# OedonLestrange42/GNURadio-WiFI-ImageTransfer

Hardware: AMD Instinct MI355X
Metric: OFDM demod throughput (complex samples/s), 802.11a RX chain sync->LLR (higher is better)
Workload: dtype f32

## Files before the change

### gnuradio-wifi-imagetransfer_amd/csrc/wr_quad.h

```cpp
#pragma once
#include "wr_device.h"
#include "wr_kernels.h"
#include <type_traits>

namespace wr {

#define WR_QLDS_SCRATCH_EQ(EQ) ((EQ) == WIFIRX_EQ_COMB ? 768 : 1200)
#define WR_QLDS_H(S)       (S)
#define WR_QLDS_TW(S)      (WR_QLDS_H(S) + 512)
#define WR_QLDS_PREV(S)    (WR_QLDS_TW(S) + 192)
#define WR_QLDS_W(S)       (WR_QLDS_PREV(S) + 48)
#define WR_QLDS_PF(S)      (WR_QLDS_W(S))
#define WR_QLDS_STAT(S)    (WR_QLDS_PF(S) + 512)
#define WR_QLDS_FLOATS(S)  (WR_QLDS_STAT(S) + 16)
#define WR_QLDS_DH(S)      (WR_QLDS_FLOATS(S))
#define WR_QLDS_FLOATS_EQ(EQ) (WR_QLDS_FLOATS(WR_QLDS_SCRATCH_EQ(EQ)) + ((EQ) == WIFIRX_EQ_COMB ? 512 : 0))

typedef float wr_f2 __attribute__((ext_vector_type(2)));
__device__ __forceinline__ float2 load_global_f2(const float2* p)
{
#if defined(__HIP_DEVICE_COMPILE__)
    const wr_f2 v = __builtin_nontemporal_load(reinterpret_cast<const __attribute__((address_space(1))) wr_f2*>(reinterpret_cast<uintptr_t>(p)));
    return make_float2(v.x, v.y);
#else
// ... 631 lines not shown
__device__ __forceinline__ void store_piece(char* p, float4 v)
{
    __builtin_nontemporal_store(wr_f4v{ v.x, v.y, v.z, v.w }, reinterpret_cast<wr_f4v*>(p));
}
__device__ __forceinline__ void store_word(uint8_t* p, uint32_t v)
{
    *reinterpret_cast<uint32_t*>(p) = v;
}

template <int NB, bool OFF32 = false, bool BF = false>
__device__ __forceinline__ void store_bins_lines(const c32 (&Y)[4], const int (&carrier)[4], bool ok, int q,
                                                 uint8_t* __restrict__ idx, float* __restrict__ llr,
                                                 uint32_t row_o, uint32_t row_l, float* stage, int row, int r)
{
    static_assert(NB == 1 || NB == 2 || NB == 4 || NB == 6, "constellation");
    constexpr int VB = BF ? 2 : 4;
    constexpr int ROWB = 48 * VB * NB, IDX0 = NB <= 2 ? (BF ? 768 : 1536) : 4 * ROWB;
    char* srow = reinterpret_cast<char*>(stage) + row * ROWB;
    uint8_t* irow = reinterpret_cast<uint8_t*>(stage) + IDX0 + row * 48;
    __builtin_amdgcn_wave_barrier();
    if (NB <= 4) {
        constexpr int ESZ = VB * NB, DUMP_L = IDX0 + 192, DUMP_I = DUMP_L + 64 * ESZ;
        const int lane = 16 * row + r;
#pragma unroll
        for (int j = 0; j < 4; j++) {
            const bool data = carrier[j] >= 0;
            char* lw = data ? srow + ESZ * carrier[j] : reinterpret_cast<char*>(stage) + DUMP_L + ESZ * lane;
            uint8_t* iw = data ? irow + carrier[j] : reinterpret_cast<uint8_t*>(stage) + DUMP_I + lane;
            if constexpr (BF) {
                if (NB == 1)      *reinterpret_cast<uint16_t*>(lw) = bf16_of(Y[j].re);
                else if (NB == 2) *reinterpret_cast<uint32_t*>(lw) = bf16_pk(Y[j].re, Y[j].im);
                else              *reinterpret_cast<uint2*>(lw) = make_uint2(bf16_pk(Y[j].re, WR_T16_2 - __builtin_fabsf(Y[j].re)),
                                                                             bf16_pk(Y[j].im, WR_T16_2 - __builtin_fabsf(Y[j].im)));
            } else
            if (NB == 1)      *reinterpret_cast<float*>(lw) = Y[j].re;
            else if (NB == 2) *reinterpret_cast<float2*>(lw) = make_float2(Y[j].re, Y[j].im);
            else              *reinterpret_cast<float4*>(lw) = make_float4(Y[j].re, WR_T16_2 - __builtin_fabsf(Y[j].re), Y[j].im, WR_T16_2 - __builtin_fabsf(Y[j].im));
            *iw = decide(Y[j], NB);
        }
    } else
#pragma unroll
    for (int j = 0; j < 4; j++) {
        const uint64_t row_bits = j == 0 ? 0xF7C0ull : j == 1 ? 0xFDFFull : j == 2 ? 0xFF7Eull : 0x07DFull;
        if (!__builtin_amdgcn_inverse_ballot_w64(row_bits * 0x0001000100010001ull)) continue;
        const float are = __builtin_fabsf(Y[j].re), aim = __builtin_fabsf(Y[j].im);
        if constexpr (BF) {
            const uint32_t ci = (uint32_t)(carrier[j] + 48 * row);
            uint32_t l12;
            if (OFF32) asm volatile("v_mul_u32_u24 %0, 12, %1" : "=v"(l12) : "v"(ci));
            else       l12 = 12u * ci;
            uint32_t* l3 = reinterpret_cast<uint32_t*>(reinterpret_cast<char*>(stage) + l12);
            l3[0] = bf16_pk(Y[j].re, WR_T64_4 - are);
            l3[1] = bf16_pk(WR_T64_2 - __builtin_fabsf(are - WR_T64_4), Y[j].im);
            l3[2] = bf16_pk(WR_T64_4 - aim, WR_T64_2 - __builtin_fabsf(aim - WR_T64_4));
            reinterpret_cast<uint8_t*>(stage)[IDX0 + ci] = decide(Y[j], NB);
            continue;
        } else
        if (NB == 1)      *reinterpret_cast<float*>(srow + 4 * carrier[j]) = Y[j].re;
        else if (NB == 2) *reinterpret_cast<float2*>(srow + 8 * carrier[j]) = make_float2(Y[j].re, Y[j].im);
        else if (NB == 4) *reinterpret_cast<float4*>(srow + 16 * carrier[j]) = make_float4(Y[j].re, WR_T16_2 - are, Y[j].im, WR_T16_2 - aim);
        else if (OFF32) {
            const uint32_t ci = (uint32_t)(carrier[j] + 48 * row);
            uint32_t l24;
            asm volatile("v_mul_u32_u24 %0, 24, %1" : "=v"(l24) : "v"(ci));
            float2* l2 = reinterpret_cast<float2*>(reinterpret_cast<char*>(stage) + l24);
            l2[0] = make_float2(Y[j].re, WR_T64_4 - are);
            l2[1] = make_float2(WR_T64_2 - __builtin_fabsf(are - WR_T64_4), Y[j].im);
            l2[2] = make_float2(WR_T64_4 - aim, WR_T64_2 - __builtin_fabsf(aim - WR_T64_4));
            reinterpret_cast<uint8_t*>(stage)[IDX0 + ci] = decide(Y[j], NB);
            continue;
        } else {
            float2* l2 = reinterpret_cast<float2*>(srow + 24 * carrier[j]);
            l2[0] = make_float2(Y[j].re, WR_T64_4 - are);
            l2[1] = make_float2(WR_T64_2 - __builtin_fabsf(are - WR_T64_4), Y[j].im);
            l2[2] = make_float2(WR_T64_4 - aim, WR_T64_2 - __builtin_fabsf(aim - WR_T64_4));
        }
        irow[carrier[j]] = decide(Y[j], NB);
    }
    __builtin_amdgcn_wave_barrier();
    constexpr int PPR = 3 * VB * NB;
    constexpr int NK = (PPR + 15) / 16, TAIL = PPR - 16 * (NK - 1);
#define WR_PIECE(k) (*reinterpret_cast<const float4*>(srow + 256 * (k) + 16 * (((k) == NK - 1 && TAIL == 8) ? (r & 7) : r)))
    const float4 p0 = WR_PIECE(0);
    float4 p1 = p0, p2 = p0, p3 = p0, p4 = p0;
    if (NK > 1) p1 = WR_PIECE(1);
    if (NK > 2) p2 = WR_PIECE(2);
    if (NK > 3) p3 = WR_PIECE(3);
    if (NK > 4) p4 = WR_PIECE(4);
#undef WR_PIECE
    const uint32_t d = reinterpret_cast<const uint32_t*>(irow)[r < 12 ? r : 0];
    __builtin_amdgcn_wave_barrier();
    if (ok) {
        char* const lb = reinterpret_cast<char*>(llr);
        const uint32_t lo = (row_l + (uint32_t)(q * 48 * NB)) * (uint32_t)VB + 16u * r;
        char* const lp = reinterpret_cast<char*>(llr) + (uint32_t)((row_l + (uint32_t)(q * 48 * NB)) * (uint32_t)VB + 16u * r);
#define WR_PIECE_AT(K) (OFF32 ? lb + (uint32_t)(lo + 256u * (K)) : lp + 256 * (K))
        if (NK > 1 || r < TAIL)            store_piece(lp, p0);
        if (NK > 2 || (NK == 2 && r < TAIL)) store_piece(WR_PIECE_AT(1), p1);
        if (NK > 3 || (NK == 3 && r < TAIL)) store_piece(WR_PIECE_AT(2), p2);
        if (NK > 4 || (NK == 4 && r < TAIL)) store_piece(WR_PIECE_AT(3), p3);
        if (NK == 5 && r < TAIL)             store_piece(WR_PIECE_AT(4), p4);
#undef WR_PIECE_AT
        if (r < 12) store_word(idx + (row_o + (uint32_t)(q * 48) + 4u * r), d);
    }
}

template <int NB, bool OFF32 = false, bool BF = false>
__device__ __forceinline__ void store_rows_x(const c32 (&Y)[4], const int (&carrier)[4], bool ok, int q,
                                             uint8_t* __restrict__ idx, float* __restrict__ llr, float2* __restrict__ car,
                                             bool has_idx, bool has_llr, bool has_car, bool csi, const float* Wl,
                                             uint32_t row_o, uint32_t row_l, float* stage, int row, int r)
{
    static_assert(NB == 1 || NB == 2 || NB == 4 || NB == 6, "constellation");
    constexpr int VB = BF ? 2 : 4;
    constexpr int ROWB = 48 * VB * NB, IDX0 = NB <= 2 ? (BF ? 768 : 1536) : 4 * ROWB;
    constexpr int PPR = 3 * VB * NB;
    constexpr int NK = (PPR + 15) / 16, TAIL = PPR - 16 * (NK - 1);
    char* srow = reinterpret_cast<char*>(stage) + row * ROWB;
    uint8_t* irow = reinterpret_cast<uint8_t*>(stage) + IDX0 + row * 48;
    float4 p0 = make_float4(0.0f, 0.0f, 0.0f, 0.0f), p1 = p0;
    if (has_idx || has_llr) {
        float w[4] = { 1.0f, 1.0f, 1.0f, 1.0f };
        if (csi) {
#pragma unroll
            for (int j = 0; j < 4; j++) w[j] = Wl[64 * j];
        }
        __builtin_amdgcn_wave_barrier();
#pragma unroll
        for (int j = 0; j < 4; j++) {
            const uint64_t row_bits = j == 0 ? 0xF7C0ull : j == 1 ? 0xFDFFull : j == 2 ? 0xFF7Eull : 0x07DFull;
            if (!__builtin_amdgcn_inverse_ballot_w64(row_bits * 0x0001000100010001ull)) continue;
            const float are = __builtin_fabsf(Y[j].re), aim = __builtin_fabsf(Y[j].im);
#define WR_WT(v) (csi ? (v) * w[j] : (v))
            if constexpr (BF) {
                if (NB == 1)      *reinterpret_cast<uint16_t*>(srow + 2 * carrier[j]) = bf16_of(WR_WT(Y[j].re));
                else if (NB == 2) *reinterpret_cast<uint32_t*>(srow + 4 * carrier[j]) = bf16_pk(WR_WT(Y[j].re), WR_WT(Y[j].im));
                else if (NB == 4) *reinterpret_cast<uint2*>(srow + 8 * carrier[j]) = make_uint2(bf16_pk(WR_WT(Y[j].re), WR_WT(WR_T16_2 - are)),
                                                                                                 bf16_pk(WR_WT(Y[j].im), WR_WT(WR_T16_2 - aim)));
                else {
                    uint32_t* l3 = reinterpret_cast<uint32_t*>(srow + 12 * carrier[j]);
                    l3[0] = bf16_pk(WR_WT(Y[j].re), WR_WT(WR_T64_4 - are));
                    l3[1] = bf16_pk(WR_WT(WR_T64_2 - __builtin_fabsf(are - WR_T64_4)), WR_WT(Y[j].im));
                    l3[2] = bf16_pk(WR_WT(WR_T64_4 - aim), WR_WT(WR_T64_2 - __builtin_fabsf(aim - WR_T64_4)));
                }
            } else
            if (NB == 1)      *reinterpret_cast<float*>(srow + 4 * carrier[j]) = WR_WT(Y[j].re);
            else if (NB == 2) *reinterpret_cast<float2*>(srow + 8 * carrier[j]) = make_float2(WR_WT(Y[j].re), WR_WT(Y[j].im));
            else if (NB == 4) *reinterpret_cast<float4*>(srow + 16 * carrier[j]) = make_float4(WR_WT(Y[j].re), WR_WT(WR_T16_2 - are), WR_WT(Y[j].im), WR_WT(WR_T16_2 - aim));
            else {
                float2* l2 = reinterpret_cast<float2*>(srow + 24 * carrier[j]);
                l2[0] = make_float2(WR_WT(Y[j].re), WR_WT(WR_T64_4 - are));
                l2[1] = make_float2(WR_WT(WR_T64_2 - __builtin_fabsf(are - WR_T64_4)), WR_WT(Y[j].im));
                l2[2] = make_float2(WR_WT(WR_T64_4 - aim), WR_WT(WR_T64_2 - __builtin_fabsf(aim - WR_T64_4)));
            }
#undef WR_WT
            irow[carrier[j]] = decide(Y[j], NB);
        }
        __builtin_amdgcn_wave_barrier();
#define WR_PIECE(k) (*reinterpret_cast<const float4*>(srow + 256 * (k) + 16 * (((k) == NK - 1 && TAIL == 8) ? (r & 7) : r)))
        p0 = WR_PIECE(0);
        float4 p2 = p0, p3 = p0, p4 = p0;
        p1 = p0;
        if (NK > 1) p1 = WR_PIECE(1);
        if (NK > 2) p2 = WR_PIECE(2);
        if (NK > 3) p3 = WR_PIECE(3);
        if (NK > 4) p4 = WR_PIECE(4);
#undef WR_PIECE
        const uint32_t d = reinterpret_cast<const uint32_t*>(irow)[r < 12 ? r : 0];
        __builtin_amdgcn_wave_barrier();
        if (ok) {
            if (has_llr) {
                char* const lb = reinterpret_cast<char*>(llr);
                const uint32_t lo = (row_l + (uint32_t)(q * 48 * NB)) * (uint32_t)VB + 16u * r;
                char* const lp = reinterpret_cast<char*>(llr) + (uint32_t)((row_l + (uint32_t)(q * 48 * NB)) * (uint32_t)VB + 16u * r);
#define WR_PIECE_AT(K) (OFF32 ? lb + (uint32_t)(lo + 256u * (K)) : lp + 256 * (K))
                if (NK > 1 || r < TAIL)            store_piece(lp, p0);
                if (NK > 2 || (NK == 2 && r < TAIL)) store_piece(WR_PIECE_AT(1), p1);
                if (NK > 3 || (NK == 3 && r < TAIL)) store_piece(WR_PIECE_AT(2), p2);
                if (NK > 4 || (NK == 4 && r < TAIL)) store_piece(WR_PIECE_AT(3), p3);
                if (NK == 5 && r < TAIL)             store_piece(WR_PIECE_AT(4), p4);
#undef WR_PIECE_AT
            }
            if (has_idx && r < 12) store_word(idx + (row_o + (uint32_t)(q * 48) + 4u * r), d);
        }
    }
    if (has_car) {
        constexpr bool QPSK_F32 = NB == 2 && !BF;
        if (!(QPSK_F32 && has_llr && !csi)) {
            char* crow = reinterpret_cast<char*>(stage) + row * 384;
            __builtin_amdgcn_wave_barrier();
#pragma unroll
            for (int j = 0; j < 4; j++) {
                const uint64_t row_bits = j == 0 ? 0xF7C0ull : j == 1 ? 0xFDFFull : j == 2 ? 0xFF7Eull : 0x07DFull;
                if (!__builtin_amdgcn_inverse_ballot_w64(row_bits * 0x0001000100010001ull)) continue;
                *reinterpret_cast<float2*>(crow + 8 * carrier[j]) = make_float2(Y[j].re, Y[j].im);
            }
            __builtin_amdgcn_wave_barrier();
            p0 = *reinterpret_cast<const float4*>(crow + 16 * r);
            p1 = *reinterpret_cast<const float4*>(crow + 256 + 16 * (r & 7));
            __builtin_amdgcn_wave_barrier();
        }
        if (ok) {
            if (OFF32) {
                char* const cb = reinterpret_cast<char*>(car);
                const uint32_t co = (row_o + (uint32_t)(q * 48)) * 8u + 16u * r;
                store_piece(cb + co, p0);
                if (r < 8) store_piece(cb + (uint32_t)(co + 256u), p1);
            } else {
                char* cp = reinterpret_cast<char*>(car) + (uint32_t)((row_o + (uint32_t)(q * 48)) * 8u + 16u * r);
                store_piece(cp, p0);
                if (r < 8) store_piece(cp + 256, p1);
            }
        }
    }
}

#define WR_HB_DATA_LO 0xFDFFF7C0u
#define WR_HB_DATA_HI 0x07DFFF7Eu

template <int NB, int B>
__device__ __forceinline__ bool decide_bit(c32 y)
{
    const float are = __builtin_fabsf(y.re), aim = __builtin_fabsf(y.im);
    if (NB == 1) return y.re > 0.0f;
    if (NB == 2) return B == 0 ? y.re > 0.0f : y.im > 0.0f;
    if (NB == 4) return B == 0 ? y.re > 0.0f : B == 1 ? are < WR_T16_2 : B == 2 ? y.im > 0.0f : aim < WR_T16_2;
    return B == 0 ? y.re > 0.0f : B == 1 ? are < WR_T64_4 : B == 2 ? (are < WR_T64_6) && (are > WR_T64_2)
         : B == 3 ? y.im > 0.0f : B == 4 ? aim < WR_T64_4 : (aim < WR_T64_6) && (aim > WR_T64_2);
}

template <int NB, int B>
__device__ __forceinline__ void plane_words(const c32 (&Y)[4], uint32_t& w0, uint32_t& w1)
{
    const uint64_t m0 = __ballot(decide_bit<NB, B>(Y[0])), m1 = __ballot(decide_bit<NB, B>(Y[1]));
    const uint64_t m2 = __ballot(decide_bit<NB, B>(Y[2])), m3 = __ballot(decide_bit<NB, B>(Y[3]));
    const uint32_t a0 = (uint32_t)m0, a1 = (uint32_t)m1, a2 = (uint32_t)m2, a3 = (uint32_t)m3;
    const uint32_t b0 = (uint32_t)(m0 >> 32), b1 = (uint32_t)(m1 >> 32), b2 = (uint32_t)(m2 >> 32), b3 = (uint32_t)(m3 >> 32);
#pragma unroll
    for (int f = 0; f < 4; f++) {
        const uint32_t p0 = f < 2 ? a0 : b0, p1 = f < 2 ? a1 : b1, p2 = f < 2 ? a2 : b2, p3 = f < 2 ? a3 : b3;
        uint32_t lo, hi;
        if (f & 1) {
            asm("s_pack_hh_b32_b16 %0, %1, %2" : "=s"(lo) : "s"(p0), "s"(p1));
            asm("s_pack_hh_b32_b16 %0, %1, %2" : "=s"(hi) : "s"(p2), "s"(p3));
        } else {
            asm("s_pack_ll_b32_b16 %0, %1, %2" : "=s"(lo) : "s"(p0), "s"(p1));
            asm("s_pack_ll_b32_b16 %0, %1, %2" : "=s"(hi) : "s"(p2), "s"(p3));
        }
        asm("v_writelane_b32 %0, %1, %2" : "+v"(w0) : "s"(lo & WR_HB_DATA_LO), "n"(16 * f));
        asm("v_writelane_b32 %0, %1, %2" : "+v"(w1) : "s"(hi & WR_HB_DATA_HI), "n"(16 * f));
    }
}

template <int NB>
__device__ __forceinline__ void store_hbits(const c32 (&Y)[4], bool ok, int q, uint32_t* __restrict__ hb, int r)
{
    uint32_t* dst = hb + (unsigned)(q * 2 * NB);
    if (NB == 1) {
        uint32_t w0 = 0, w1 = 0;
        plane_words<1, 0>(Y, w0, w1);
        if (ok && r == 0) *reinterpret_cast<uint2*>(dst) = make_uint2(w0, w1);
    } else {
        uint4 w = make_uint4(0u, 0u, 0u, 0u);
        plane_words<NB, 0>(Y, w.x, w.y);
        plane_words<NB, 1>(Y, w.z, w.w);
        if (ok && r == 0) *reinterpret_cast<uint4*>(dst) = w;
        if (NB >= 4) {
            plane_words<NB, 2>(Y, w.x, w.y);
            plane_words<NB, (NB >= 4 ? 3 : 0)>(Y, w.z, w.w);
            if (ok && r == 0) *reinterpret_cast<uint4*>(dst + 4) = w;
        }
        if (NB == 6) {
            plane_words<NB, (NB == 6 ? 4 : 0)>(Y, w.x, w.y);
            plane_words<NB, (NB == 6 ? 5 : 0)>(Y, w.z, w.w);
            if (ok && r == 0) *reinterpret_cast<uint4*>(dst + 8) = w;
        }
    }
}

__device__ __forceinline__ c32 point_of(unsigned idx, int n_bpsc)
{
    c32 p;
    if (n_bpsc == 1) { p.re = (idx & 1) ? 1.0f : -1.0f; p.im = 0.0f; return p; }
    if (n_bpsc == 2) {
        p.re = (idx & 1) ? WR_LEVEL_QPSK : -WR_LEVEL_QPSK;
        p.im = (idx & 2) ? WR_LEVEL_QPSK : -WR_LEVEL_QPSK;
        return p;
    }
    if (n_bpsc == 4) {
        const float l = WR_T16_2 * 0.5f;
        float ar = (idx & 2) ? l : 3.0f * l, ai = (idx & 8) ? l : 3.0f * l;
        p.re = (idx & 1) ? ar : -ar;
        p.im = (idx & 4) ? ai : -ai;
        return p;
    }
    const float l = WR_T64_2 * 0.5f;
    unsigned r = (idx >> 1) & 3, q = (idx >> 4) & 3;
    unsigned kr = ((r & 1) << 1) | (r >> 1), kq = ((q & 1) << 1) | (q >> 1);
    float ar = (kr == 0 ? 7.0f : kr == 1 ? 5.0f : kr == 2 ? 1.0f : 3.0f) * l;
    float ai = (kq == 0 ? 7.0f : kq == 1 ? 5.0f : kq == 2 ? 1.0f : 3.0f) * l;
    p.re = (idx & 1) ? ar : -ar;
    p.im = (idx & 8) ? ai : -ai;
    return p;
}

template <int EQ, bool HB, bool XK, bool BF = false>
__device__ __forceinline__ void frames_quad(const QuadSeed& seed, const DemodParams& prm, float* qlds, int lane,
                                            const DemodOut& dout)
{
    wifirx_frame* __restrict__ frames = dout.frames;
    uint8_t* __restrict__ idx_all = dout.idx;
    float* __restrict__ llr_all = dout.llr;
    float2* __restrict__ car_all = dout.carrier;
    float2* __restrict__ csi_all = dout.csi;
    float4* __restrict__ stat_all = dout.sym_stats;
    uint32_t* __restrict__ hb_all = dout.hbits;
    constexpr bool LMS = EQ == WIFIRX_EQ_LMS, COMB = EQ == WIFIRX_EQ_COMB, STA = EQ == WIFIRX_EQ_STA;
    constexpr int QS = WR_QLDS_SCRATCH_EQ(EQ);
    constexpr bool DIV = EQ != WIFIRX_EQ_LS;
    const int row = lane >> 4, r = lane & 15;
    const bool  has = seed.out >= 0 && seed.x != nullptr && seed.t >= 0;
    const long  t16 = seed.t - 16;
    const uint64_t has_m = __ballot(has);
    const int has_l = has_m ? (int)__builtin_ctzll(has_m) : 0;
    const uint64_t xv = has ? reinterpret_cast<uint64_t>(seed.x + t16) : 0ull;
    const uint64_t xf = ((uint64_t)(uint32_t)__builtin_amdgcn_readlane((int)(xv >> 32), has_l) << 32) |
                        (uint32_t)__builtin_amdgcn_readlane((int)xv, has_l);
    const float2* xb = has ? seed.x + t16 : reinterpret_cast<const float2*>(xf);
    const int   m_lo = has ? (int)(t16 < 0 ? -t16 : 0) : 0;
    const long  m_hi_l = seed.n_samp - t16;
    const int   m_hi = has ? (int)(m_hi_l > 0x7fffff00l ? 0x7fffff00l : m_hi_l) : 0;
    const int   L = (int)seed.L;
    const bool  lo_zero = __all(m_lo == 0 && L <= m_hi && (!has || m_hi >= 64));
    const int   out = (int)seed.out;
    const int   trig = (int)seed.t;
    const float cfo_c = seed.cfo_c, cfo_f = seed.cfo_f;
    const int   fs = seed.fs;
    uint32_t flags = seed.flags;
    bool alive = (out >= 0) && (flags & WIFIRX_F_SYNC);
    const double bw = prm.bandwidth, fc = prm.frequency;
    const double two_pi = 2 * 3.14159265358979323846;
    const double tag = (double)cfo_c - (double)cfo_f;
    const float eps0 = (float)(tag * bw / (two_pi * fc));
    const float er_scale = (float)(bw / (two_pi * fc * 80));
    float d_er = 0.0f;
    const double theta_d = (double)cfo_f - (double)cfo_c;
    const unsigned long long Qp = (unsigned long long)(long long)__builtin_rint(theta_d * WR_TWO_OVER_PI_D * 4611686018427387904.0);
    constexpr bool QP_LDS = EQ != WIFIRX_EQ_LS;
    constexpr int PVS = QP_LDS ? 6 : 4;
    uint2* const qpl = reinterpret_cast<uint2*>(qlds + WR_QLDS_PREV(WR_QLDS_SCRATCH_EQ(EQ))) + PVS * (lane >> 4) + 4;
    if (QP_LDS && (lane & 15) == 0) *qpl = make_uint2((uint32_t)Qp, (uint32_t)(Qp >> 32));
    c32 u16;
    {
        const unsigned long long q16 = Qp * 16ull;
        sp_sincos_q((uint32_t)(q16 >> 32), (uint32_t)q16, u16.im, u16.re);
    }
    c32 u80;
    {
        const unsigned long long q80 = Qp * 80ull;
        sp_sincos_q((uint32_t)(q80 >> 32), (uint32_t)q80, u80.im, u80.re);
    }
    c32 wbase = { 1.0f, 0.0f };
    const float rp_bpsk = sp_recip(1.0f);
    const float rp_qpsk = sp_recip(fma_(WR_LEVEL_QPSK, WR_LEVEL_QPSK, WR_LEVEL_QPSK * WR_LEVEL_QPSK));
    int n_sym = 0, n_bpsc = 1, n_out = 0, enc = 0, psdu_len = 0;
    bool have_signal = false, want_llr = false;
    float snr = 0.0f;

    float2* twl = reinterpret_cast<float2*>(qlds + WR_QLDS_TW(QS));
    if (row == 0) {
#pragma unroll
        for (int j = 1; j < 4; j++) {
            int e1 = (j * r) & 63, e2 = (j * (r & 3) * 4) & 63;
            twl[(j - 1) * 16 + r] = make_float2(WR_TWIDDLE64[2 * e1], WR_TWIDDLE64[2 * e1 + 1]);
            twl[(j + 2) * 16 + r] = make_float2(WR_TWIDDLE64[2 * e2], WR_TWIDDLE64[2 * e2 + 1]);
        }
    }
    float* stl = qlds + WR_QLDS_STAT(QS) + 4 * row;
    if (stat_all != nullptr && r < 4) stl[r] = 0.0f;
    float2* Hl = reinterpret_cast<float2*>(qlds + WR_QLDS_H(QS)) + lane;
    float2* pvl = reinterpret_cast<float2*>(qlds + WR_QLDS_PREV(QS)) + PVS * row;
    float* Wl = qlds + WR_QLDS_W(QS) + lane;
    float2* DHl = reinterpret_cast<float2*>(qlds + (COMB ? WR_QLDS_DH(QS) : WR_QLDS_H(QS))) + lane;
    float cw[4] = { 0.0f, 0.0f, 0.0f, 0.0f }, cu[4] = { 0.0f, 0.0f, 0.0f, 0.0f };
    if (COMB) {
#pragma unroll
        for (int j = 0; j < 4; j++) { cw[j] = WR_COMB_W[r + 16 * j]; cu[j] = WR_COMB_U[r + 16 * j]; }
    }
    auto sta_inv_of = [&](int j) __attribute__((always_inline)) -> float {
        const uint64_t m3 = j == 0 ? 0x0040ull : j == 3 ? 0x0400ull : 0ull;
        const uint64_t m4 = j == 0 ? 0x0080ull : j == 1 ? 0xC000ull : j == 2 ? 0x0006ull : 0x0200ull;
        float v = 0x1.99999ap-3f;
        v = __builtin_amdgcn_inverse_ballot_w64(m4 * 0x0001000100010001ull) ? 0.25f : v;
        if (m3) v = __builtin_amdgcn_inverse_ballot_w64(m3 * 0x0001000100010001ull) ? 0x1.555556p-2f : v;
        return v;
    };
    int carrier0[4];
#pragma unroll
    for (int j = 0; j < 4; j++) {
        const int i = r + 16 * j;
        const bool data = (i >= 6 && i <= 58 && i != 11 && i != 25 && i != 32 && i != 39 && i != 53);
        carrier0[j] = data ? (i - 6 - (i > 11) - (i > 25) - (i > 32) - (i > 39) - (i > 53)) : -1;
    }
    __builtin_amdgcn_wave_barrier();
    constexpr bool TP_PAD = EQ != WIFIRX_EQ_COMB;
    float2* ql = reinterpret_cast<float2*>(qlds) + (TP_PAD ? 144 * row : 128 * (row >> 1) + 16 * (row & 1));
    const int m4 = 4 * (r & 3), c2 = r >> 2;
    const size_t per = (size_t)prm.max_sym * 48;
    const uint64_t have_out = __ballot(out >= 0);
    const int out_base = have_out ? __builtin_amdgcn_readlane(out, (int)__builtin_ctzll(have_out)) : 0;
    const uint32_t row_o = out >= 0 ? (uint32_t)(out - out_base) * (uint32_t)per : 0u;
    const uint32_t row_l = row_o * prm.llr_bits;
    uint8_t* idx = idx_all ? idx_all + (size_t)out_base * per : nullptr;
    float*   llr = llr_all ? llr_all + (size_t)out_base * per * prm.llr_bits : nullptr;
    if constexpr (BF)
        llr = llr_all ? reinterpret_cast<float*>(reinterpret_cast<uint16_t*>(llr_all) + (size_t)out_base * per * prm.llr_bits) : nullptr;
    float2*  car = car_all ? car_all + (size_t)out_base * per : nullptr;
    const bool lines_ok = (reinterpret_cast<uintptr_t>(idx) & 3) == 0 && (reinterpret_cast<uintptr_t>(llr) & 15) == 0 && ((per * prm.llr_bits) & 3) == 0;

    uint64_t polw = WR_POLARITY_NEG_LO;
    int poln = 64;
    int polhi = 0;
    float t4 = WR_T4_64F[0];
    const float* t4_next = WR_T4_64F + 1;
    int s_end = 0;
    int nbu_all = 0;
    bool plain_all = false;
    bool x_idx = false, x_llr = false, x_car = false, x_csi = false;
    uint32_t pf_voff0 = 0, pf_voff1 = 0;
    const float2* pf_next = nullptr;
    int pf_end = 0;
    bool pf_row = false;
    int pf_nst = 0;
    const uint32_t pf_m0 = (uint32_t)__builtin_amdgcn_readfirstlane((int)(uint32_t)reinterpret_cast<uintptr_t>(qlds + WR_QLDS_PF(QS)));
    const uint32_t pf_m1 = (uint32_t)__builtin_amdgcn_readfirstlane((int)(pf_m0 + 1024u));
    auto pf_issue = [&](float dep) __attribute__((always_inline)) {
        asm volatile("s_mov_b32 m0, %0\n\ts_nop 0\n\tglobal_load_lds_dwordx4 %2, %4\n\t"
                     "s_mov_b32 m0, %1\n\ts_nop 0\n\tglobal_load_lds_dwordx4 %3, %4"
                     :: "s"(pf_m0), "s"(pf_m1), "v"(pf_voff0), "v"(pf_voff1), "s"(pf_next), "v"(dep) : "memory", "m0");
        pf_next += 80;
    };
    auto pf_setup = [&](uint64_t has_data, int s0) __attribute__((always_inline)) -> bool {
        const int first = (int)__builtin_ctzll(has_data);
        const bool mine = s_end > 3;
        pf_end = __builtin_amdgcn_readlane(s_end, first);
        pf_row = mine;
        const uint64_t xbv = reinterpret_cast<uint64_t>(xb);
        const uint64_t xref = ((uint64_t)(uint32_t)__builtin_amdgcn_readlane((int)(xbv >> 32), first) << 32) |
                              (uint32_t)__builtin_amdgcn_readlane((int)xbv, first);
        const int64_t dist = (int64_t)(xbv - xref) / (int64_t)sizeof(float2);
        if (!__all(!mine || (s_end == pf_end && dist >= 0 && dist < (1 << 26)))) return false;
        const int c_own = (int)dist + fs;
        const int c_ref = __builtin_amdgcn_readlane(c_own, first);
        const int c = mine ? c_own : c_ref;
        const int c0 = __builtin_amdgcn_readlane(c, 0), c1 = __builtin_amdgcn_readlane(c, 16);
        const int c2 = __builtin_amdgcn_readlane(c, 32), c3 = __builtin_amdgcn_readlane(c, 48);
        pf_voff0 = (uint32_t)((lane < 32 ? c0 : c1) + 2 * (lane & 31)) * 8u;
        pf_voff1 = (uint32_t)((lane < 32 ? c2 : c3) + 2 * (lane & 31)) * 8u;
        pf_next = reinterpret_cast<const float2*>(xref) + (128 + 80 * (s0 - 2) + 16);
        __builtin_amdgcn_wave_barrier();
        pf_issue(0.0f);
        asm volatile("s_waitcnt vmcnt(0)" ::: "memory");
        return true;
    };
    auto symbol = [&](auto data_c, auto nb_c, auto x_c, auto p_c, const int s) __attribute__((always_inline)) -> bool {
        constexpr bool DATA = decltype(data_c)::value;
        constexpr int NBC = decltype(nb_c)::value;
        constexpr bool XC = decltype(x_c)::value;
        constexpr bool PC = decltype(p_c)::value;
        const int off0 = fs + ((!DATA && s < 2) ? 64 * s : 128 + 80 * (s - 2) + 16);
        bool act;
        if (DATA) {
            act = PC ? pf_row : s < s_end;
        } else {
            act = alive && (s <= n_sym + 2);
            if (act && (off0 + 64 > L || (s > 2 && (s - 3) >= (int)prm.max_sym))) {
                flags |= WIFIRX_F_TRUNCATED;
                alive = false;
                act = false;
            }
        }
        if (!(DATA && PC) && !__any(act)) return false;

        c32 v[4], cur[4];
        {
            if (PC) {
                constexpr int NST = ((BF ? 6 : 12) * (NBC ? NBC : 1) + 15) / 16 + 1 + (HB ? ((NBC ? NBC : 1) + 1) / 2 : 0);
                if (XC) {
                    switch (pf_nst) {
#define WR_W(N) case N: asm volatile("s_waitcnt vmcnt(" #N ")" ::: "memory"); break;
                    WR_W(1) WR_W(2) WR_W(3) WR_W(4) WR_W(5) WR_W(6) WR_W(7) WR_W(8) WR_W(9) WR_W(10) WR_W(11)
#undef WR_W
                    default: asm volatile("s_waitcnt vmcnt(0)" ::: "memory"); break;
                    }
                } else
                asm volatile("s_waitcnt vmcnt(%0)" :: "n"(NST) : "memory");
                const float2* pb = reinterpret_cast<const float2*>(qlds + WR_QLDS_PF(QS)) + 64 * row + r;
#pragma unroll
                for (int j = 0; j < 4; j++) { const float2 t = pb[16 * j]; cur[j] = { t.x, t.y }; }
            } else
            if (NBC != 0 || lo_zero) {
                const float2* p = xb + ((act ? off0 : 0) + r);
#pragma unroll
                for (int j = 0; j < 4; j++) { const float2 t = load_global_f2(p + 16 * j); cur[j] = { t.x, t.y }; }
            } else {
#pragma unroll
                for (int j = 0; j < 4; j++) cur[j] = load_y(xb, off0 + r + 16 * j, m_lo, act ? m_hi : 0);
            }
        }
        {
            if ((!DATA && s < 2) || ((s - 1) & 7) == 0) {
                unsigned long long qp = Qp;
                if (DATA && QP_LDS) { const uint2 q2 = *qpl; qp = ((unsigned long long)q2.y << 32) | q2.x; }
                const unsigned long long ph = qp * (unsigned long long)(unsigned)(off0 + r);
                sp_sincos_q((uint32_t)(ph >> 32), (uint32_t)ph, wbase.im, wbase.re);
            } else {
                wbase = sp_cmul(wbase, u80);
            }
            c32 w = wbase;
#pragma unroll
            for (int j = 0; j < 4; j++) {
                v[j] = sp_cmul(cur[j], w);
                w = sp_cmul(w, u16);
            }
            if (PC && s + 1 < pf_end) pf_issue(v[3].re);
        }
        bfly4_reg(v[0], v[1], v[2], v[3]);
#pragma unroll
        for (int j = 0; j < 4; j++) {
            c32 y = v[0];
            if (j) { float2 w = twl[(j - 1) * 16 + r]; y = sp_cmul(v[j], c32{ w.x, w.y }); }
            ql[TP_PAD ? 33 * j + m4 + c2 : 32 * j + m4 + (j ^ c2)] = make_float2(y.re, y.im);
        }
        __builtin_amdgcn_wave_barrier();
#pragma unroll
        for (int j = 0; j < 4; j++) {
            float2 t = ql[TP_PAD ? 33 * c2 + m4 + j : 32 * c2 + m4 + (c2 ^ j)];
            v[j] = { t.x, t.y };
        }
        __builtin_amdgcn_wave_barrier();
        bfly4_reg(v[0], v[1], v[2], v[3]);
#pragma unroll
        for (int j = 0; j < 4; j++) {
            c32 y = v[0];
            if (j) { float2 w = twl[(j + 2) * 16 + r]; y = sp_cmul(v[j], c32{ w.x, w.y }); }
            ql[TP_PAD ? 33 * j + 4 * c2 + (r & 3) : 32 * j + 4 * c2 + (j ^ (r & 3))] = make_float2(y.re, y.im);
        }
        __builtin_amdgcn_wave_barrier();
#pragma unroll
        for (int j = 0; j < 4; j++) {
            float2 t = ql[TP_PAD ? 33 * c2 + m4 + j : 32 * c2 + m4 + (c2 ^ j)];
            v[j] = { t.x, t.y };
        }
        __builtin_amdgcn_wave_barrier();
        bfly4_reg(v[0], v[1], v[2], v[3]);
        c32 X[4] = { v[2], v[3], v[0], v[1] };

        {
            const float kf = t4 * (eps0 + d_er);
            if (DATA) { t4 = PC ? load_const_f(t4_next) : *t4_next; t4_next++; }
            else { t4 = WR_T4_64F[s + 1]; t4_next = WR_T4_64F + (s + 2); }
            c32 b;
            sp_sincos_small(kf * (float)(r - 16), b.im, b.re);
            const c32 b0 = row_bcast<0>(b), step = { b0.re, -b0.im };
            const c32 q0 = sp_cmul(b, b0), q2 = sp_cmul(b, step), q3 = sp_cmul(q2, step);
            X[0] = sp_cmul(X[0], q0);
            X[1] = sp_cmul(X[1], b);
            X[2] = sp_cmul(X[2], q2);
            X[3] = sp_cmul(X[3], q3);
        }
        c32 X11 = row_bcast<11>(X[0]), X25 = row_bcast<9>(X[1]), X39 = row_bcast<7>(X[2]), X53 = row_bcast<5>(X[3]);
        uint32_t sgn = 0;
        c32 S, cur0, cur1, cur2, cur3;
        float er = 0.0f;
        if (DATA || s >= 2) {
            sgn = (uint32_t)polw << 31;
            polw >>= 1;
            if (__builtin_expect(--poln == 0, 0)) { polhi ^= 1; polw = polhi ? WR_POLARITY_NEG_HI : WR_POLARITY_NEG_LO; poln = 64 - polhi; }
            S = cflip(csub(cadd(cadd(X11, X39), X25), X53), sgn);
            cur0 = cflip(X11, sgn);
            cur1 = cflip(X25, sgn);
            cur2 = cflip(X39, sgn);
            cur3 = cflip(X53, sgn ^ 0x80000000u);
            const float2 q0 = pvl[0], q1 = pvl[1], q2 = pvl[2], q3 = pvl[3];
            const c32 prev0 = { q0.x, q0.y }, prev1 = { q1.x, q1.y }, prev2 = { q2.x, q2.y }, prev3 = { q3.x, q3.y };
            c32 acc = cadd(cadd(cadd(sp_conj_mul(prev0, cur0), sp_conj_mul(prev1, cur1)),
                                sp_conj_mul(prev2, cur2)), sp_conj_mul(prev3, cur3));
            er = sp_atan2(acc.im, acc.re) * er_scale;
        } else {
            S = cadd(cadd(csub(X11, X25), X39), X53);
            cur0 = X11; cur1 = cneg(X25); cur2 = X39; cur3 = X53;
        }
        __builtin_amdgcn_wave_barrier();
        if (r == 0) {
            pvl[0] = make_float2(cur0.re, cur0.im); pvl[1] = make_float2(cur1.re, cur1.im);
            pvl[2] = make_float2(cur2.re, cur2.im); pvl[3] = make_float2(cur3.re, cur3.im);
        }
        __builtin_amdgcn_wave_barrier();
        {
            float n2 = fma_(S.im, S.im, S.re * S.re);
            float inv = sp_rsqrt(n2);
            float cs = (n2 > 0.0f) ? S.re * inv : 1.0f;
            float sn = (n2 > 0.0f) ? -(S.im * inv) : 0.0f;
#pragma unroll
            for (int j = 0; j < 4; j++) X[j] = sp_rot(X[j], sn, cs);
        }
        if (DATA || s >= 2) d_er = fma_(0.1f, er, 0.9f * d_er);
        if (COMB) {
            c32 n1 = row_bcast<11>(X[0]), n2 = row_bcast<9>(X[1]), n3 = row_bcast<7>(X[2]), n4 = row_bcast<5>(X[3]);
            if (!DATA && s < 2) n2 = cneg(n2);
            else { n1 = cflip(n1, sgn); n2 = cflip(n2, sgn); n3 = cflip(n3, sgn); n4 = cflip(n4, sgn ^ 0x80000000u); }
            const c32 sum = cadd(cadd(cadd(n1, n2), n3), n4);
            const c32 n0 = { 0.25f * sum.re, 0.25f * sum.im };
            const c32 node[6] = { n0, n1, n2, n3, n4, n0 };
            const int edge[4] = { 11, 25, 39, 53 };
#pragma unroll
            for (int j = 0; j < 4; j++) {
                const bool lo = (r + 16 * j) <= edge[j];
                const c32 a = lo ? node[j] : node[j + 1], b = lo ? node[j + 1] : node[j + 2];
                const float hr = fma_(b.re, cw[j], a.re * cu[j]), hi = fma_(b.im, cw[j], a.im * cu[j]);
                if (!DATA && s == 0) DHl[64 * j] = make_float2(hr, hi);
                else {
                    const float2 o = DHl[64 * j];
                    DHl[64 * j] = make_float2(0.8f * o.x + 0.2f * hr, 0.8f * o.y + 0.2f * hi);
                }
            }
        }
        if (!DATA && s == 0) {
#pragma unroll
            for (int j = 0; j < 4; j++) Hl[64 * j] = make_float2(X[j].re, X[j].im);
        } else if (!DATA && s == 1) {
            float nv[4], sv[4];
#pragma unroll
            for (int j = 0; j < 4; j++) {
                const float2 h0 = Hl[64 * j];
                const c32 Hj = { h0.x, h0.y };
                c32 d = csub(Hj, X[j]), u = cadd(Hj, X[j]);
                const int i = r + 16 * j;
                const bool usedj = (i >= 6 && i <= 58 && i != 32);
                nv[j] = usedj ? fma_(d.im, d.im, d.re * d.re) : 0.0f;
                sv[j] = usedj ? fma_(u.im, u.im, u.re * u.re) : 0.0f;
                float g = 0.5f * WR_LTS_FREQ[i];
                const float hr = u.re * g, hi = u.im * g;
                const float dd = fma_(hi, hi, hr * hr);
                if (prm.llr_csi) Wl[64 * j] = usedj ? dd : 0.0f;
                if (csi_all && usedj && act) csi_all[(size_t)out * 52 + (i - 6 - (i > 32))] = make_float2(hr, hi);
                if (LMS || STA) {
                    Hl[64 * j] = usedj ? make_float2(hr, hi) : make_float2(1.0f, 0.0f);
                } else if (COMB) {
                } else {
                    Hl[64 * j] = usedj ? make_float2(hr / dd, -hi / dd) : make_float2(0.0f, 0.0f);
                }
                nv[j] = row_xor_sum16(nv[j]);
                sv[j] = row_xor_sum16(sv[j]);
            }
            float n01 = nv[0] + nv[1], n23 = nv[2] + nv[3], s01 = sv[0] + sv[1], s23 = sv[2] + sv[3];
            float noise = n01 + n23, signal = s01 + s23;
            if (act) snr = sp_snr_db(signal, noise);
        } else {
            c32 Y[4];
            int carrier[4];
            c32 HU[4];
            const bool const_mag = (LMS || STA) && (NBC != 0 ? NBC <= 2 : __all((!DATA && s == 2) || n_bpsc <= 2));
#pragma unroll
            for (int j = 0; j < 4; j++) {
                carrier[j] = carrier0[j];
                if (NBC == 0) asm volatile("" : "+v"(carrier[j]));
                Y[j] = { 0.0f, 0.0f };
                HU[j] = X[j];
                if (!(STA && NBC == 0) || carrier[j] >= 0) {
                    const float2 g0 = DHl[64 * j];
                    if (DIV) {
                        const float rd = sp_recip(fma_(g0.y, g0.y, g0.x * g0.x));
                        Y[j].re = fma_(X[j].im, g0.y, X[j].re * g0.x) * rd;
                        Y[j].im = fma_(X[j].im, g0.x, -(X[j].re * g0.y)) * rd;
                        if (LMS || STA) {
                            const int nbl = NBC != 0 ? NBC : (!DATA && s == 2) ? 1 : n_bpsc;
                            const c32 pt = point_of(decide(Y[j], nbl), nbl);
                            float rp;
                            if (const_mag) rp = nbl == 1 ? rp_bpsk : rp_qpsk;
                            else           rp = sp_recip(fma_(pt.im, pt.im, pt.re * pt.re));
                            const float tr = fma_(X[j].im, pt.im, X[j].re * pt.re) * rp;
                            const float ti = fma_(X[j].im, pt.re, -(X[j].re * pt.im)) * rp;
                            if (LMS) Hl[64 * j] = make_float2(0.5f * g0.x + 0.5f * tr, 0.5f * g0.y + 0.5f * ti);
                            HU[j] = { tr, ti };
                        }
                    } else {
                        Y[j] = sp_cmul(X[j], c32{ g0.x, g0.y });
                    }
                }
            }
            if (STA) {
                if (r == 11) HU[0] = cflip(X[0], sgn);
                if (r == 9)  HU[1] = cflip(X[1], sgn);
                if (r == 7)  HU[2] = cflip(X[2], sgn);
                if (r == 5)  HU[3] = cflip(X[3], sgn ^ 0x80000000u);
                float2* hu = reinterpret_cast<float2*>(qlds) + 68 * row + 2;
                __builtin_amdgcn_wave_barrier();
#pragma unroll
                for (int j = 0; j < 4; j++) {
                    const int i = r + 16 * j;
                    const bool usedj = (i >= 6 && i <= 58 && i != 32);
                    hu[i] = usedj ? make_float2(HU[j].re, HU[j].im) : make_float2(0.0f, 0.0f);
                }
                if (r < 2) { hu[r - 2] = make_float2(0.0f, 0.0f); hu[64 + r] = make_float2(0.0f, 0.0f); }
                __builtin_amdgcn_wave_barrier();
#pragma unroll
                for (int j = 0; j < 4; j++) {
                    const int i = r + 16 * j;
                    const bool usedj = (i >= 6 && i <= 58 && i != 32);
                    const float2 v0 = hu[i - 2], v1 = hu[i - 1], v2 = hu[i], v3 = hu[i + 1], v4 = hu[i + 2];
                    const c32 sum = cadd(cadd(cadd(cadd(c32{ v0.x, v0.y }, c32{ v1.x, v1.y }), c32{ v2.x, v2.y }), c32{ v3.x, v3.y }),
                                         c32{ v4.x, v4.y });
                    const float2 o = Hl[64 * j];
                    const float inv = sta_inv_of(j);
                    if (act && usedj) Hl[64 * j] = make_float2(0.5f * o.x + 0.5f * (sum.re * inv), 0.5f * o.y + 0.5f * (sum.im * inv));
                }
                __builtin_amdgcn_wave_barrier();
            }
            if (!DATA && s == 2) {
                uint64_t bal[4];
#pragma unroll
                for (int j = 0; j < 4; j++) bal[j] = __ballot(carrier[j] >= 0 && Y[j].re > 0.0f);
                const uint64_t actmask = __ballot(act);
                const int dsrc = lane < 48 ? 3 * (lane & 15) + (lane >> 4) : 63;
                uint64_t de[4];
#pragma unroll
                for (int f = 0; f < 4; f++) {
                    uint64_t b = 0;
#pragma unroll
                    for (int j = 0; j < 4; j++) b |= ((bal[j] >> (16 * f)) & 0xffffull) << (16 * j);
                    const uint64_t cm = ((b >> 6) & 0x1full) | (((b >> 12) & 0x1fffull) << 5) |
                                        (((b >> 26) & 0x3full) << 18) | (((b >> 33) & 0x3full) << 24) |
                                        (((b >> 40) & 0x1fffull) << 30) | (((b >> 54) & 0x1full) << 43);
                    de[f] = __ballot(((cm >> dsrc) & 1ull) != 0);
                }
                uint32_t sig4[4];
                viterbi_signal4(de, lane, sig4);
#pragma unroll
                for (int f = 0; f < 4; f++) {
                    if (!((actmask >> (16 * f)) & 1)) continue;
                    const uint32_t sig = sig4[f];
                    int e = 0, len = 0;
                    bool ok = parse_signal(sig, e, len);
                    if (row == f) {
                        if (!ok) {
                            alive = false;
                        } else {
                            const int nbpsc_tab[8] = { 1, 1, 2, 2, 4, 4, 6, 6 };
                            const int ndbps_tab[8] = { 24, 36, 48, 72, 96, 144, 192, 216 };
                            have_signal = true;
                            enc = e;
                            psdu_len = len;
                            n_bpsc = nbpsc_tab[e];
                            int nd = ndbps_tab[e];
                            n_sym = (16 + 8 * len + 6 + nd - 1) / nd;
                            flags |= WIFIRX_F_SIGNAL;
                            want_llr = (llr != nullptr) && ((int)prm.llr_bits >= n_bpsc);
                            if (want_llr) flags |= WIFIRX_F_LLR;
                        }
                    }
                }
            } else {
                const int q = s - 3;
                const bool has_idx = idx_all != nullptr, has_car = car_all != nullptr;
                int out_l = out;
                if (HB) asm volatile("" : "+v"(out_l));
                const uint64_t act_m = __ballot(act);
                const bool settled = DATA && nbu_all > 0;
                const int nbu = settled ? nbu_all : __builtin_amdgcn_readlane(n_bpsc, act_m ? (int)__builtin_ctzll(act_m) : 0);
                const bool uniform = settled || (act_m & ~__ballot(n_bpsc == nbu)) == 0;
                const float w1[4] = { 1.0f, 1.0f, 1.0f, 1.0f };
                const bool csi = prm.llr_csi != 0 && llr_all != nullptr;
                const bool no_bins = HB && !has_idx && !has_car && llr_all == nullptr;
#define WR_STORE(NB, OK)                                                                                        \
                { if (no_bins) { }                                                                                      \
                  else if (csi) { const float wq[4] = { Wl[0], Wl[64], Wl[128], Wl[192] };                                   \
                             store_bins<NB, true, false, BF>(Y, carrier, OK, q, idx, car, llr, has_idx, has_car, want_llr, wq, row_o, row_l); }  \
                  else if (DATA && plain_all) store_bins<NB, false, true, BF>(Y, carrier, OK, q, idx, car, llr, true, false, true, w1, row_o, row_l); \
                  else     store_bins<NB, false, false, BF>(Y, carrier, OK, q, idx, car, llr, has_idx, has_car, want_llr, w1, row_o, row_l); \
                  if (HB) { __builtin_amdgcn_sched_barrier(0);                                                          \
                            store_hbits<NB>(Y, OK, q, hb_all + (size_t)(unsigned)out_l * (prm.max_sym * 12u), r); } }
                if (NBC != 0 && XC) {
                    store_rows_x<(NBC ? NBC : 1), EQ != WIFIRX_EQ_LS, BF>(Y, carrier, act, q, idx, llr, car, x_idx, x_llr, x_car, x_csi, Wl, row_o, row_l, qlds, row, r);
                    if (HB) { __builtin_amdgcn_sched_barrier(0);
                              store_hbits<(NBC ? NBC : 1)>(Y, act, q, hb_all + (size_t)(unsigned)out_l * (prm.max_sym * 12u), r); }
                } else if (NBC != 0) {
                    if ((NBC <= 2 || !COMB) && (PC || lines_ok))
                        store_bins_lines<(NBC ? NBC : 1), EQ != WIFIRX_EQ_LS, BF>(Y, carrier, act, q, idx, llr, row_o, row_l, qlds, row, r);
                    else
                    store_bins<(NBC ? NBC : 1), false, true, BF>(Y, carrier, act, q, idx, car, llr, true, false, true, w1, row_o, row_l);
                    if (HB) { __builtin_amdgcn_sched_barrier(0);
                              store_hbits<(NBC ? NBC : 1)>(Y, act, q, hb_all + (size_t)(unsigned)out_l * (prm.max_sym * 12u), r); }
                } else if (uniform) {
                    if (nbu == 1)      WR_STORE(1, act)
                    else if (nbu == 2) WR_STORE(2, act)
                    else if (nbu == 4) WR_STORE(4, act)
                    else               WR_STORE(6, act)
                } else {
                    WR_STORE(1, act && n_bpsc == 1)
                    WR_STORE(2, act && n_bpsc == 2)
                    WR_STORE(4, act && n_bpsc == 4)
                    WR_STORE(6, act && n_bpsc == 6)
                }
#undef WR_STORE
                if ((NBC == 0 || XC) && stat_all != nullptr) {
                    float p1 = 0.0f, p2 = 0.0f, p4 = 0.0f;
#pragma unroll
                    for (int j = 0; j < 4; j++) {
                        const float m2 = fma_(Y[j].im, Y[j].im, Y[j].re * Y[j].re);
                        const bool d = carrier[j] >= 0;
                        const float a1 = d ? __builtin_sqrtf(m2) : 0.0f, a2 = d ? m2 : 0.0f, a4 = d ? m2 * m2 : 0.0f;
                        p1 = j ? p1 + a1 : a1; p2 = j ? p2 + a2 : a2; p4 = j ? p4 + a4 : a4;
                    }
                    p1 = row_xor_sum16(p1); p2 = row_xor_sum16(p2); p4 = row_xor_sum16(p4);
                    if (act && r == 0) { stl[0] += p1; stl[1] += p2; stl[2] += p4; }
                }
                if (act) n_out = q + 1;
            }
        }
        return true;
    };
    {
        int s = 0;
        bool more = true;
        typedef std::integral_constant<int, 0> nb_any;
        typedef std::false_type no_x;
        typedef std::false_type no_p;
        for (; more && s < 3; s++) more = symbol(std::false_type{}, nb_any{}, no_x{}, no_p{}, s);
#if defined(WR_ABLATE) && WR_ABLATE == 3
        more = false;
#endif
        uint64_t has_data = 0;
        if (more) {
            const int s_fit = 2 + (L - fs - 208) / 80, s_max = (int)prm.max_sym + 2;
            const int s_lim = s_fit < s_max ? s_fit : s_max;
            const bool cut = alive && s_lim < n_sym + 2;
            if (cut) { flags |= WIFIRX_F_TRUNCATED; alive = false; }
            s_end = (alive || cut) ? (cut ? s_lim : n_sym + 2) + 1 : 0;
            has_data = __ballot(s_end > 3);
            const int nb_first = has_data ? __builtin_amdgcn_readlane(n_bpsc, (int)__builtin_ctzll(has_data)) : 0;
            nbu_all = (has_data & ~__ballot(n_bpsc == nb_first)) == 0 ? nb_first : 0;
            plain_all = idx_all != nullptr && car_all == nullptr && (has_data & ~__ballot(want_llr)) == 0;
        }
        const bool special = !XK && more && nbu_all > 0 && plain_all && !(prm.llr_csi != 0 && llr_all != nullptr) &&
                             lo_zero && stat_all == nullptr;
        bool pf = false;
        bool loops = false;
        if constexpr (XK) {
            const uint64_t llr_rows = has_data & __ballot(want_llr);
            loops = more && nbu_all > 0 && !special && lo_zero && (llr_rows == 0 || llr_rows == has_data) &&
                    (reinterpret_cast<uintptr_t>(idx) & 3) == 0 && (reinterpret_cast<uintptr_t>(llr) & 15) == 0 &&
                    (reinterpret_cast<uintptr_t>(car) & 15) == 0 && ((per * prm.llr_bits) & 3) == 0 && (per & 1) == 0;
            x_idx = idx_all != nullptr;
            x_llr = llr_rows != 0;
            x_car = car_all != nullptr;
            x_csi = prm.llr_csi != 0 && llr_all != nullptr;
            if (loops && !x_csi && (x_llr || x_car) && (!COMB || nbu_all <= 2)) {
                pf = pf_setup(has_data, s);
                const int nk = ((BF ? 6 : 12) * nbu_all + 15) / 16;
                pf_nst = (x_llr ? nk : 0) + (x_idx ? 1 : 0) + (x_car ? 2 : 0) + (HB ? (nbu_all + 1) / 2 : 0);
            }
        } else {
            loops = special;
            if (special && (!COMB || nbu_all <= 2) && lines_ok) pf = pf_setup(has_data, s);
        }
        typedef std::integral_constant<bool, XK> x_c;
        typedef std::true_type data;
        typedef std::true_type with_p;
        typedef std::integral_constant<int, 1> nb1;
        typedef std::integral_constant<int, 2> nb2;
        typedef std::integral_constant<int, 4> nb4;
        typedef std::integral_constant<int, 6> nb6;
        if (pf && nbu_all == 1)                  { for (; s < pf_end; s++) (void)symbol(data{}, nb1{}, x_c{}, with_p{}, s); more = false; }
        else if (pf && nbu_all == 2)             { for (; s < pf_end; s++) (void)symbol(data{}, nb2{}, x_c{}, with_p{}, s); more = false; }
        else if (!COMB && pf && nbu_all == 4)    { for (; s < pf_end; s++) (void)symbol(data{}, nb4{}, x_c{}, with_p{}, s); more = false; }
        else if (!COMB && pf && nbu_all == 6)    { for (; s < pf_end; s++) (void)symbol(data{}, nb6{}, x_c{}, with_p{}, s); more = false; }
        else if (loops && nbu_all == 1)          for (; more; s++) more = symbol(data{}, nb1{}, x_c{}, no_p{}, s);
        else if (loops && nbu_all == 2)          for (; more; s++) more = symbol(data{}, nb2{}, x_c{}, no_p{}, s);
        else if (!COMB && loops && nbu_all == 4) for (; more; s++) more = symbol(data{}, nb4{}, x_c{}, no_p{}, s);
        else if (!COMB && loops && nbu_all == 6) for (; more; s++) more = symbol(data{}, nb6{}, x_c{}, no_p{}, s);
        else                                     for (; more; s++) more = symbol(data{}, nb_any{}, no_x{}, no_p{}, s);
    }
    if (r == 0 && out >= 0) {
        wifirx_frame fr;
        if (have_signal && n_out == n_sym) flags |= WIFIRX_F_COMPLETE;
        bool sync = (flags & WIFIRX_F_SYNC) != 0;
        fr.flags = flags;
        fr.trigger = trig;
        fr.frame_start = sync ? fs : 0;
        fr.cfo_coarse = (flags & WIFIRX_F_DETECTED) ? cfo_c : 0.0f;
        fr.cfo_fine = sync ? cfo_f : 0.0f;
        fr.snr_db = snr;
        fr.psdu_len = (uint16_t)psdu_len;
        fr.encoding = (uint8_t)enc;
        fr.n_bpsc = have_signal ? (uint8_t)n_bpsc : 0;
        fr.n_sym = (uint16_t)n_sym;
        fr.n_sym_out = (uint16_t)n_out;
        frames[out] = fr;
        if (stat_all != nullptr) stat_all[out] = make_float4(stl[0], stl[1], stl[2], 0.0f);
    }
}

}
```

Measured before the change: 425.9 billion.

## Software-pipeline LS data-symbol loop across FFT front and equalizer back stages

Adds a pipelined per-symbol loop for the LS equalizer prefetch path that interleaves the next symbol's FFT stages with the current symbol's phase tracking, equalization and LLR store. The aim is to hide LDS and ALU latency and the dependency chain of the pilot tracking by overlapping independent work from two symbols. It is selected at compile time for NB values 1, 2, 4 and 6 through a bitmask macro. In exchange it raises register pressure, which may reduce occupancy, and it duplicates logic from the generic symbol lambda.

```diff
diff --git a/gnuradio-wifi-imagetransfer_amd/csrc/wr_quad.h b/gnuradio-wifi-imagetransfer_amd/csrc/wr_quad.h
--- a/gnuradio-wifi-imagetransfer_amd/csrc/wr_quad.h
+++ b/gnuradio-wifi-imagetransfer_amd/csrc/wr_quad.h
@@ -957,6 +957,14 @@
     p.re = (idx & 1) ? ar : -ar;
     p.im = (idx & 8) ? ai : -ai;
     return p;
+}
+
+#ifndef WR_PIPELINE_NB
+#define WR_PIPELINE_NB 0x56
+#endif
+__host__ __device__ constexpr bool wr_pipelined(int eq, bool xk, bool bf, int nb)
+{
+    return eq == WIFIRX_EQ_LS && !xk && !bf && ((WR_PIPELINE_NB >> nb) & 1) != 0;
 }
 
 template <int EQ, bool HB, bool XK, bool BF = false>
@@ -1476,6 +1484,145 @@
         }
         return true;
     };
+    auto data_pipelined = [&](auto nb_c, int& s) __attribute__((always_inline)) {
+        constexpr int NB = decltype(nb_c)::value;
+        static_assert(EQ == WIFIRX_EQ_LS && !XK, "the pipelined loop is written for the LS instances of the usual output set");
+        constexpr int NST = ((BF ? 6 : 12) * NB + 15) / 16 + 1 + (HB ? (NB + 1) / 2 : 0);
+        const float2* const pb = reinterpret_cast<const float2*>(qlds + WR_QLDS_PF(QS)) + 64 * row + r;
+        const bool act = pf_row;
+        c32 v[4];
+        c32 X[4];
+        uint32_t sgn = 0;
+        c32 S = { 0.0f, 0.0f };
+        float2 tw2[3], gq[4];
+        auto front_a = [&](const int sf) __attribute__((always_inline)) {
+            asm volatile("s_waitcnt vmcnt(%0)" :: "n"(NST) : "memory");
+            c32 cur[4];
+#pragma unroll
+            for (int j = 0; j < 4; j++) { const float2 t = pb[16 * j]; cur[j] = { t.x, t.y }; }
+            float2 tw1[3];
+#pragma unroll
+            for (int j = 0; j < 3; j++) tw1[j] = twl[j * 16 + r];
+            __builtin_amdgcn_wave_barrier();
+            if (((sf - 1) & 7) == 0) {
+                const unsigned long long ph = Qp * (unsigned long long)(unsigned)(fs + 128 + 80 * (sf - 2) + 16 + r);
+                sp_sincos_q((uint32_t)(ph >> 32), (uint32_t)ph, wbase.im, wbase.re);
+            } else {
+                wbase = sp_cmul(wbase, u80);
+            }
+            c32 w = wbase;
+#pragma unroll
+            for (int j = 0; j < 4; j++) {
+                v[j] = sp_cmul(cur[j], w);
+                w = sp_cmul(w, u16);
+            }
+            if (sf + 1 < pf_end) pf_issue(v[3].re);
+            bfly4_reg(v[0], v[1], v[2], v[3]);
+#pragma unroll
+            for (int j = 0; j < 4; j++) {
+                c32 y = v[0];
+                if (j) { const float2 w1 = tw1[j - 1]; y = sp_cmul(v[j], c32{ w1.x, w1.y }); }
+                ql[33 * j + m4 + c2] = make_float2(y.re, y.im);
+            }
+            __builtin_amdgcn_wave_barrier();
+#pragma unroll
+            for (int j = 0; j < 4; j++) { const float2 t = ql[33 * c2 + m4 + j]; v[j] = { t.x, t.y }; }
+#pragma unroll
+            for (int j = 0; j < 3; j++) tw2[j] = twl[(j + 3) * 16 + r];
+            __builtin_amdgcn_wave_barrier();
+        };
+        auto front_b = [&]() __attribute__((always_inline)) {
+            bfly4_reg(v[0], v[1], v[2], v[3]);
+#pragma unroll
+            for (int j = 0; j < 4; j++) {
+                c32 y = v[0];
+                if (j) { const float2 w1 = tw2[j - 1]; y = sp_cmul(v[j], c32{ w1.x, w1.y }); }
+                ql[33 * j + 4 * c2 + (r & 3)] = make_float2(y.re, y.im);
+            }
+            __builtin_amdgcn_wave_barrier();
+#pragma unroll
+            for (int j = 0; j < 4; j++) { const float2 t = ql[33 * c2 + m4 + j]; v[j] = { t.x, t.y }; }
+#pragma unroll
+            for (int j = 0; j < 4; j++) gq[j] = Hl[64 * j];
+            __builtin_amdgcn_wave_barrier();
+        };
+        auto front_c = [&]() __attribute__((always_inline)) {
+            bfly4_reg(v[0], v[1], v[2], v[3]);
+            X[0] = v[2]; X[1] = v[3]; X[2] = v[0]; X[3] = v[1];
+        };
+        auto back_a = [&]() __attribute__((always_inline)) {
+            sgn = (uint32_t)polw << 31;
+            polw >>= 1;
+            if (__builtin_expect(--poln == 0, 0)) { polhi ^= 1; polw = polhi ? WR_POLARITY_NEG_HI : WR_POLARITY_NEG_LO; poln = 64 - polhi; }
+            const float kf = t4 * (eps0 + d_er);
+            t4 = load_const_f(t4_next);
+            t4_next++;
+            c32 b;
+            sp_sincos_small(kf * (float)(r - 16), b.im, b.re);
+            const c32 b0 = row_bcast<0>(b), step = { b0.re, -b0.im };
+            const c32 q0 = sp_cmul(b, b0), q2 = sp_cmul(b, step), q3 = sp_cmul(q2, step);
+            X[0] = sp_cmul(X[0], q0);
+            X[1] = sp_cmul(X[1], b);
+            X[2] = sp_cmul(X[2], q2);
+            X[3] = sp_cmul(X[3], q3);
+        };
+        auto back_b = [&]() __attribute__((always_inline)) {
+            const c32 X11 = row_bcast<11>(X[0]), X25 = row_bcast<9>(X[1]), X39 = row_bcast<7>(X[2]), X53 = row_bcast<5>(X[3]);
+            S = cflip(csub(cadd(cadd(X11, X39), X25), X53), sgn);
+            const c32 cur0 = cflip(X11, sgn), cur1 = cflip(X25, sgn), cur2 = cflip(X39, sgn), cur3 = cflip(X53, sgn ^ 0x80000000u);
+            const float2 p0 = pvl[0], p1 = pvl[1], p2 = pvl[2], p3 = pvl[3];
+            const c32 prev0 = { p0.x, p0.y }, prev1 = { p1.x, p1.y }, prev2 = { p2.x, p2.y }, prev3 = { p3.x, p3.y };
+            const c32 acc = cadd(cadd(cadd(sp_conj_mul(prev0, cur0), sp_conj_mul(prev1, cur1)),
+                                      sp_conj_mul(prev2, cur2)), sp_conj_mul(prev3, cur3));
+            const float er = sp_atan2(acc.im, acc.re) * er_scale;
+            __builtin_amdgcn_wave_barrier();
+            if (r == 0) {
+                pvl[0] = make_float2(cur0.re, cur0.im); pvl[1] = make_float2(cur1.re, cur1.im);
+                pvl[2] = make_float2(cur2.re, cur2.im); pvl[3] = make_float2(cur3.re, cur3.im);
+            }
+            __builtin_amdgcn_wave_barrier();
+            d_er = fma_(0.1f, er, 0.9f * d_er);
+        };
+        c32 Y[4];
+        auto back_c = [&]() __attribute__((always_inline)) {
+            const float n2 = fma_(S.im, S.im, S.re * S.re);
+            const float inv = sp_rsqrt(n2);
+            const float cs = (n2 > 0.0f) ? S.re * inv : 1.0f;
+            const float sn = (n2 > 0.0f) ? -(S.im * inv) : 0.0f;
+#pragma unroll
+            for (int j = 0; j < 4; j++) {
+                const float2 g0 = gq[j];
+                Y[j] = sp_cmul(sp_rot(X[j], sn, cs), c32{ g0.x, g0.y });
+            }
+        };
+        auto back_d = [&](const int sb) __attribute__((always_inline)) {
+            const int q = sb - 3;
+            int out_l = out;
+            if (HB) asm volatile("" : "+v"(out_l));
+            store_bins_lines<NB, false, BF>(Y, carrier0, act, q, idx, llr, row_o, row_l, qlds, row, r);
+            if (HB) { __builtin_amdgcn_sched_barrier(0);
+                      store_hbits<NB>(Y, act, q, hb_all + (size_t)(unsigned)out_l * (prm.max_sym * 12u), r); }
+            if (act) n_out = q + 1;
+        };
+        front_a(s);
+        front_b();
+        front_c();
+        asm volatile("s_waitcnt vmcnt(0)" ::: "memory");
+        for (; s + 1 < pf_end; s++) {
+            front_a(s + 1);
+            back_a();
+            back_b();
+            front_b();
+            back_c();
+            front_c();
+            back_d(s);
+        }
+        back_a();
+        back_b();
+        back_c();
+        back_d(s);
+        s++;
+    };
     {
         int s = 0;
         bool more = true;
@@ -1527,10 +1674,15 @@
         typedef std::integral_constant<int, 2> nb2;
         typedef std::integral_constant<int, 4> nb4;
         typedef std::integral_constant<int, 6> nb6;
-        if (pf && nbu_all == 1)                  { for (; s < pf_end; s++) (void)symbol(data{}, nb1{}, x_c{}, with_p{}, s); more = false; }
-        else if (pf && nbu_all == 2)             { for (; s < pf_end; s++) (void)symbol(data{}, nb2{}, x_c{}, with_p{}, s); more = false; }
-        else if (!COMB && pf && nbu_all == 4)    { for (; s < pf_end; s++) (void)symbol(data{}, nb4{}, x_c{}, with_p{}, s); more = false; }
-        else if (!COMB && pf && nbu_all == 6)    { for (; s < pf_end; s++) (void)symbol(data{}, nb6{}, x_c{}, with_p{}, s); more = false; }
+#define WR_PF_LOOP(NBT)                                                                                         \
+        { if constexpr (wr_pipelined(EQ, XK, BF, NBT::value)) data_pipelined(NBT{}, s);                         \
+          else for (; s < pf_end; s++) (void)symbol(data{}, NBT{}, x_c{}, with_p{}, s);                         \
+          more = false; }
+        if (pf && nbu_all == 1)                  WR_PF_LOOP(nb1)
+        else if (pf && nbu_all == 2)             WR_PF_LOOP(nb2)
+        else if (!COMB && pf && nbu_all == 4)    WR_PF_LOOP(nb4)
+        else if (!COMB && pf && nbu_all == 6)    WR_PF_LOOP(nb6)
+#undef WR_PF_LOOP
         else if (loops && nbu_all == 1)          for (; more; s++) more = symbol(data{}, nb1{}, x_c{}, no_p{}, s);
         else if (loops && nbu_all == 2)          for (; more; s++) more = symbol(data{}, nb2{}, x_c{}, no_p{}, s);
         else if (!COMB && loops && nbu_all == 4) for (; more; s++) more = symbol(data{}, nb4{}, x_c{}, no_p{}, s);
```

Result: no change. 428.9 billion (median of 6 runs) (+0.7%).
